# peterropac/Aegolius

Measured on AMD Instinct MI355X. Metric: Mpoints/sec SDF eval, 1024^3 grid, 10-prim smooth-union tree, higher is better.
Workload: dtype f32

## Files before the change

__graft_entry__.py:

```python
import os
import subprocess
import sys

ROOT = os.path.dirname(os.path.abspath(__file__))
CSRC = os.path.join(ROOT, "aegolius_amd", "csrc")
LIB = os.path.join(ROOT, "aegolius_amd", "libsdfk.so")
HELPER = os.path.join(ROOT, "aegolius_amd", "sdfk_rtc_helper")
HELPER_SRC = os.path.join(CSRC, "sdfk_rtc_helper.c")
SOURCES = ["sdfk.hip", "sdfk_codegen.cpp"]
DEPS = SOURCES + ["sdfk_device.h", "sdfk_access.h", "sdfk_codegen.h", "sdfk_ops.def", "sdfk_jit.inc", "sdfk_launch.inc", "sdfk_gridops.inc", "sdfk_fieldops.inc", "sdfk_vector.inc", "sdfk_vecdev.h",
                  "sdfk_hosttree.inc", "sdfk_lcwg.inc", "sdfk_dual.inc", "sdfk_project.inc", "sdfk_dualdev.h", "sdfk_adjoint.inc", "sdfk_points.inc", "sdfk_mesh.inc", "sdfk_slices.inc", "sdfk_topology.inc", "sdfk_rays.inc", "sdfk_raydev.h", "sdfk_raycull.h", "sdfk_interpfield.h", "sdfk_occupancy.inc", "sdfk_occdev.h", "sdfk_moments.inc", "sdfk_momdev.h", "sdfk_redistance.inc", "sdfk_boxdev.h", "sdfk_enclosure.inc", "embed.py",
                  os.path.join("..", "_mctable.py"),
                  os.path.join("..", "..", "include", "sdfk.h")]
HIPCC_FLAGS = ["--offload-arch=gfx950", "-O3", "-ffp-contract=off", "-fno-honor-nans", "-mno-amdgpu-ieee", "-std=c++17",
               "-fPIC", "-shared"]


def _stale():
    if not os.path.exists(LIB):
        return True
    t = os.path.getmtime(LIB)
    return any(os.path.getmtime(os.path.join(CSRC, d)) > t for d in DEPS)


def _write_mesh_table():
    import importlib.util
    spec = importlib.util.spec_from_file_location("_sdfk_mctable", os.path.join(ROOT, "aegolius_amd", "_mctable.py"))
    mod = importlib.util.module_from_spec(spec)
    spec.loader.exec_module(mod)
    mod.write_inc(os.path.join(CSRC, "sdfk_mesh_table.inc"))


def build(force=False):
    if ROOT not in sys.path:
        sys.path.insert(0, ROOT)
    if force or _stale():
        hipcc = os.environ.get("HIPCC") or "/opt/rocm/bin/hipcc"
        if not os.path.exists(hipcc):
            hipcc = "hipcc"
        sys.path.insert(0, CSRC)
        try:
            import embed
            embed.main()
        finally:
# ... 66 lines not shown
```

aegolius_amd/csrc/embed.py:

```python
import os
import sys


def main(out_path=None):
    here = os.path.dirname(os.path.abspath(__file__))
    out_path = out_path or os.path.join(here, "sdfk_embedded.inc")
    parts = []
    for var, name in (("kEmbeddedDevice", "sdfk_device.h"), ("kEmbeddedAccess", "sdfk_access.h"),
                      ("kEmbeddedVecdev", "sdfk_vecdev.h"), ("kEmbeddedRaydev", "sdfk_raydev.h"),
                      ("kEmbeddedRaycull", "sdfk_raycull.h"), ("kEmbeddedOccdev", "sdfk_occdev.h"),
                      ("kEmbeddedMomdev", "sdfk_momdev.h")):
        text = open(os.path.join(here, name)).read()
        assert ')SDFKSRC"' not in text
        parts.append('static const char %s[] = R"SDFKSRC(\n%s\n)SDFKSRC";\n' % (var, text))
    new = "// generated by embed.py - do not edit\n" + "\n".join(parts)
    if not os.path.exists(out_path) or open(out_path).read() != new:
        with open(out_path, "w") as f:
            f.write(new)
    return out_path


if __name__ == "__main__":
    main(*sys.argv[1:])
```

aegolius_amd/csrc/sdfk.hip:

```cpp
#include <hip/hip_runtime.h>
#include <hip/hiprtc.h>

#include <chrono>
#include <algorithm>
#include <atomic>
#include <cmath>
#include <condition_variable>
#include <cstdio>
#include <cstdlib>
#include <cstring>
#include <deque>
#include <functional>
#include <map>
#include <memory>
#include <mutex>
#include <thread>
#include <string>
#include <variant>
#include <vector>
#include <dirent.h>
#include <dlfcn.h>
#include <fcntl.h>
#include <signal.h>
#include <spawn.h>
// ... 676 lines not shown
    const double step = delta / div;
    for (int64_t i = 0; i < n; ++i) {
        volatile double t = (step != 0.0) ? (double)i * step : ((double)i / div) * delta;
        out[i] = (float)(t + lo);
    }
    out[n - 1] = (float)hi;
    return 0;
}

struct AxisTables {
    float* d = nullptr;
    ~AxisTables() {
        if (d) (void)hipFree(d);
    }
};

static int upload_axes(const float* ax0, int64_t n0, const float* ax1, int64_t n1, const float* ax2, int64_t n2,
                       hipStream_t stream, AxisTables* t, SrcGrid* g, int64_t start) {
    if (!ax0 || !ax1 || !ax2 || n0 < 1 || n1 < 1 || n2 < 1) return fail(-1, "grid axes missing or empty");
    if (n1 > 0x7fffffff || n2 > 0x7fffffff) return fail(-1, "grid axis too long");
    HIPCHK(hipMalloc(&t->d, (size_t)(n0 + n1 + n2) * sizeof(float)));
    HIPCHK(hipMemcpyAsync(t->d, ax0, (size_t)n0 * sizeof(float), hipMemcpyHostToDevice, stream));
    HIPCHK(hipMemcpyAsync(t->d + n0, ax1, (size_t)n1 * sizeof(float), hipMemcpyHostToDevice, stream));
    HIPCHK(hipMemcpyAsync(t->d + n0 + n1, ax2, (size_t)n2 * sizeof(float), hipMemcpyHostToDevice, stream));
    g->ax0 = t->d;
    g->ax1 = t->d + n0;
    g->ax2 = t->d + n0 + n1;
    g->n1 = (unsigned)n1;
    g->n2 = (unsigned)n2;
    g->start = start;
    return 0;
}

extern "C" int sdfk_eval_grid_aux(sdfk_program* p, const float* ax0, int64_t n0, const float* ax1, int64_t n1,
                                  const float* ax2, int64_t n2, int64_t start, int64_t count, const float* d_aux, int n_aux,
                                  int64_t aux_stride, float* d_out, void* stream, int mode) {
    if (!p || !d_out) return fail(-1, "sdfk_eval_grid_aux: null pointer");
    if (start < 0 || count < 0 || start + count > n0 * n1 * n2) return fail(-1, "sdfk_eval_grid_aux: range outside the grid");
    if (n_aux < p->n_aux) return fail(-1, "sdfk_eval_grid_aux: the program reads more auxiliary fields than were passed");
    AxisTables t;
    SrcGrid g;
    int rc = upload_axes(ax0, n0, ax1, n1, ax2, n2, (hipStream_t)stream, &t, &g, start);
    if (rc) return rc;
    EvalCall c = grid_call(p, &g, count, d_out, stream, mode, aligned16(d_out));
    c.aux = d_aux;
    c.aux_stride = aux_stride;
    rc = run(c);
    if (rc) return rc;
    HIPCHK(hipStreamSynchronize((hipStream_t)stream));
    return 0;
}
extern "C" int sdfk_eval_grid(sdfk_program* p, const float* ax0, int64_t n0, const float* ax1, int64_t n1,
                              const float* ax2, int64_t n2, int64_t start, int64_t count, float* d_out, void* stream,
                              int mode) {
    if (!d_out) return fail(-1, "sdfk_eval_grid: null output");
    if (start < 0 || count < 0 || start + count > n0 * n1 * n2) return fail(-1, "sdfk_eval_grid: range outside the grid");
    if (!p) return fail(-1, "null program");
    return sdfk_eval_grid_aux(p, ax0, n0, ax1, n1, ax2, n2, start, count, nullptr, p->n_aux, 0, d_out, stream, mode);
}

extern "C" int sdfk_eval_grid_host(sdfk_program* p, const float* ax0, int64_t n0, const float* ax1, int64_t n1,
                                   const float* ax2, int64_t n2, int64_t start, int64_t count, float* out, int device,
                                   int mode) {
    if (!p) return fail(-1, "null program");
    if (count < 0 || (count > 0 && !out)) return fail(-1, "sdfk_eval_grid_host: bad arguments");
    if (start < 0 || start + count > n0 * n1 * n2) return fail(-1, "sdfk_eval_grid_host: range outside the grid");
    if (count == 0) return 0;
    HIPCHK(hipSetDevice(device));
    int64_t chunk = std::min<int64_t>(count, (int64_t)1 << 27);
    const int64_t grow = n2 > 1 ? n2 : n1;
    if (start % grow == 0 && chunk > grow) chunk = chunk / grow * grow;
    float* d_out = nullptr;
    HIPCHK(hipMalloc(&d_out, (size_t)chunk * sizeof(float)));
    AxisTables t;
    SrcGrid g;
// ... 379 lines not shown
```

aegolius_amd/csrc/sdfk_codegen.cpp:

```cpp
#include "sdfk_codegen.h"

#include <algorithm>
#include <cstdio>
#include <cstring>
#include <map>
#include <set>

#include "sdfk_embedded.inc"

std::string sdfk_vector_prelude() { return std::string(kEmbeddedDevice) + "\n" + kEmbeddedVecdev + "\n"; }

static const char kWrappers[] = R"SDFKW(
template <int VEC, typename SRC>
static __device__ __forceinline__ void sdfk_body(const float* __restrict__ PRM, const float* __restrict__ TAB,
                                                 const SRC& src, long long off, long long n,
                                                 float* __restrict__ out, const float* __restrict__ aux,
                                                 long long aux_stride, unsigned* __restrict__ flags, unsigned thr) {
    const long long block_base = (long long)sdfk_bx() * (SDFK_BLOCK * VEC);
    const unsigned lane_off = sdfk_tx() * VEC;
#ifdef SDFK_FLAGS                                              // the flag-writing build of this flavour (its own code object:
    {                                                          // carried as a run-time branch it cost the field kernels registers)
        const bool active = block_base + lane_off < n;
        unsigned nib = 0u;
        if (active) {
// ... 1455 lines not shown
        bool run = false;
        unsigned rec = 0u;
        if (j < cnt) {
            rec = listed ? cp.cand[off + j] : sdfk_member_record(j);
            const float e = SDFK_CHAIN_SGN * sdfk_leaf_rec<float>(rec, c, PRM, TAB);
            run = !(e - m >= thr0 + 1e-6f * fabsf(e));
        }
        const unsigned long long bits = __ballot(run);
        if (run) cp.cand[at + n_out + (unsigned)__builtin_popcountll(bits & ((1ull << lane) - 1ull))] = rec;
        n_out += (unsigned)__builtin_popcountll(bits);
    }
    if (lane == 0) cp.span[cell] = make_uint2(at, total);
}
#else
#define SDFK_CELLS_KARG
#endif
)SDFKR";
static const char kRowsArray[] = R"SDFKR(
extern "C" __global__ __launch_bounds__(64 * SDFK_RWAVES) SDFK_ROWS_ATTR void sdfk_spec_r(
    const float* __restrict__ PRM, const float* __restrict__ TAB, const float* __restrict__ co, long long stride,
    sdfk_rowgeom g, float* __restrict__ out, unsigned* __restrict__ flags, unsigned thr SDFK_CELLS_KARG) {
    const SrcArray s = {co, stride};
    sdfk_rows_kernel(PRM, TAB, s, g, out, flags, thr SDFK_CELLS_PASS);
}
#ifdef SDFK_CELLS
extern "C" __global__ __launch_bounds__(256) void sdfk_spec_cells(
    const float* __restrict__ PRM, const float* __restrict__ TAB, const float* __restrict__ co, long long stride,
    sdfk_rowgeom g, sdfk_cellpass cp) {
    const SrcArray s = {co, stride};
    sdfk_cells_kernel(PRM, TAB, s, g, cp);
}
#endif
)SDFKR";
static const char kRowsGrid[] = R"SDFKR(
// the same on a regular grid expanded from three per-axis tables (no coordinate array: 4 B/point); the slab
// starts at a row boundary and out[0] is its first point
extern "C" __global__ __launch_bounds__(64 * SDFK_RWAVES) void sdfk_spec_rg(
    const float* __restrict__ PRM, const float* __restrict__ TAB, SrcGrid s, sdfk_rowgeom g, float* __restrict__ out,
    unsigned* __restrict__ flags, unsigned thr SDFK_CELLS_KARG) {
    sdfk_rows_kernel(PRM, TAB, s, g, out, flags, thr SDFK_CELLS_PASS);
}
#ifdef SDFK_CELLS
extern "C" __global__ __launch_bounds__(256) void sdfk_spec_cellsg(
    const float* __restrict__ PRM, const float* __restrict__ TAB, SrcGrid s, sdfk_rowgeom g, sdfk_cellpass cp) {
    sdfk_cells_kernel(PRM, TAB, s, g, cp);
}
#endif
)SDFKR";
static const char kRowsMask[] = R"SDFKR(
// test aid: the skip masks (two 64-bit words per brick: sites 0-31, 32-63; bit 2k = first operand of site k
// skipped, bit 2k+1 = second) followed by the "uniform rows" flag in a third word
extern "C" __global__ __launch_bounds__(64 * SDFK_RWAVES) void sdfk_spec_rmask(
    const float* __restrict__ PRM, const float* __restrict__ TAB, const float* __restrict__ co, long long stride,
    sdfk_rowgeom g, unsigned long long* __restrict__ masks) {
    __shared__ __attribute__((aligned(16))) sdfk_rowmeta meta;
    const SrcArray s = {co, stride};
    unsigned rb, c;
    sdfk_rows_prepare(PRM, TAB, s, g, &meta, sdfk_bx(), rb, c);
    const unsigned q = sdfk_bx() * SDFK_RNBRICK + sdfk_tx();
    if (sdfk_tx() < SDFK_RNBRICK && q < g.nbricks) {
        masks[3ull * q] = meta.mask[0][sdfk_tx()];
        masks[3ull * q + 1] = meta.mask[1][sdfk_tx()];
        masks[3ull * q + 2] = meta.uniform[sdfk_tx()];
    }
}
)SDFKR";

namespace {

struct Gen {
    const sdfk_opinfo* ops;
    int n_ops;
    const uint32_t* code;
// ... 886 lines not shown
        g.s += kSpecField;
        g.s += flavour == SDFK_FL_SPANS ? kSpans : flavour == SDFK_FL_SECONDARY ? kSecondary : kRays;
        if (chain) {
            g.s += "\n#ifndef SDFK_RAYS_CULL_MIN_LEAVES\n#define SDFK_RAYS_CULL_MIN_LEAVES 64    // (measured: DESIGN 4.14 has the table)\n#endif\n"
                   "#if SDFK_NLEAF >= SDFK_RAYS_CULL_MIN_LEAVES\n";
            g.s += kWaveHelpers;
            g.s += kEmbeddedRaycull;
            g.s += flavour == SDFK_FL_SPANS ? kSpansCullKernels : flavour == SDFK_FL_SECONDARY ? kSecondaryCullKernels : kRaysCullKernels;
            g.s += "#endif\n";
        }
        return g.s;
    }
    if (chain_analyse(g, result_reg, sites_all)) {
        const bool flat2 = flavour == SDFK_FL_ROWS2D_ARRAY || flavour == SDFK_FL_ROWS2D_GRID;
        g.emit_chain_common();
        if (plain) {
            g.s += kWrappers;
            if (all || flavour == SDFK_FL_PLAIN_ARRAY) g.s += kWrappersArray;
            if (all || flavour == SDFK_FL_PLAIN_GRID) g.s += kWrappersGrid;
        }
        if (all || flat2 || flavour == SDFK_FL_ROWS_ARRAY || flavour == SDFK_FL_ROWS_GRID || flavour == SDFK_FL_ROWS_MASK) {
            g.s += kWaveHelpers;
            if (flat2) g.s += "\n#define SDFK_FLAT 1\n";
            g.s += "\n#define SDFK_NP 4\n#define SDFK_EACH _Pragma(\"unroll\") for (int q = 0; q < SDFK_NP; ++q)\n"
                   "#define SDFK_NMASK 2\n"
                   "#define SDFK_SIMT 1\n#define SDFK_NSUB 1\n"
                   "#ifndef SDFK_CELLS_MIN_LEAVES\n#define SDFK_CELLS_MIN_LEAVES 64\n#endif\n"
                   "#if !defined(SDFK_NO_CELLS) && SDFK_NLEAF > SDFK_CELLS_MIN_LEAVES\n#define SDFK_CELLS 1\n#endif\n"
                   "#ifndef SDFK_LEAF_UNROLL\n#define SDFK_LEAF_UNROLL _Pragma(\"unroll 4\")\n#endif\n";
            g.s += kSimtGeometry;
            g.emit_probe_leaves(g.leaves.size() >= 128, true);
            g.s += kRowsKernel;
            if (all || flavour == SDFK_FL_ROWS_ARRAY || flavour == SDFK_FL_ROWS2D_ARRAY) g.s += kRowsArray;
            if (all || flavour == SDFK_FL_ROWS_GRID || flavour == SDFK_FL_ROWS2D_GRID) g.s += kRowsGrid;
        }
        return g.s;
    }
    if (plain) {
        g.s += "\ntemplate <typename T> static __device__ __forceinline__ T sdfk_point(V3T<T> C_0, "
               "const float* __restrict__ PRM, const float* __restrict__ TAB, const float* __restrict__ AUX, "
               "long long AUXS) {\n";
        g.declare("V3T<T>", "T", false);
        for (size_t i = 0; i < n_instr; ++i) g.instr(i, "    ");
        snprintf(buf, sizeof buf, "    return V_%d;\n}\n", result_reg);
        g.s += buf;
        g.s += kWrappers;
        if (all || flavour == SDFK_FL_PLAIN_ARRAY) g.s += kWrappersArray;
        if (all || flavour == SDFK_FL_PLAIN_GRID) g.s += kWrappersGrid;
    }
    if (tile || rowk) g.s += kWaveHelpers;
    if (tile) {
        std::vector<size_t> order(sites.size());
        for (size_t i = 0; i < order.size(); ++i) order[i] = i;
        std::stable_sort(order.begin(), order.end(), [&](size_t x, size_t y) {
            return sites[x].comb - sites[x].a0 > sites[y].comb - sites[y].a0;
        });
        order.resize(std::min<size_t>(order.size(), 31));
        std::sort(order.begin(), order.end());
        std::vector<sdfk_cullsite> flat;
        for (size_t i : order) flat.push_back(sites[i]);
        g.sites = &flat;
        g.find_roots();
        snprintf(buf, sizeof buf, "\n#define SDFK_NROOT %d\n", g.n_root > 0 ? g.n_root : 1);
        g.s += buf;
        g.emit_probe();
        g.emit_culled(result_reg);
        g.s += kTileKernel;
// ... 8 lines not shown
        g.n_root = 0;
        g.find_roots();
        if (flat) g.s += "\n#define SDFK_FLAT 1\n";
        g.s += "\n#define SDFK_NP 4\n#define SDFK_EACH _Pragma(\"unroll\") for (int q = 0; q < SDFK_NP; ++q)\n";
        {
            char nm[64];
            snprintf(nm, sizeof nm, "#define SDFK_NMASK %zu\n", std::max<size_t>(2, (sites.size() + 31) / 32));
            g.s += nm;
        }
        g.s += "#ifndef SDFK_CHAIN_LOOP_MIN\n#define SDFK_CHAIN_LOOP_MIN 100000   // chains of at least this many sites run as a loop over the levels that survive\n#endif\n"
               "// the even bits of x, packed into the low 32 bits (wave-uniform: scalar unit)\n"
               "static __device__ __forceinline__ unsigned long long sdfk_even_bits(unsigned long long x) {\n"
               "    x &= 0x5555555555555555ull;\n"
               "    x = (x | (x >> 1)) & 0x3333333333333333ull;\n"
               "    x = (x | (x >> 2)) & 0x0f0f0f0f0f0f0f0full;\n"
               "    x = (x | (x >> 4)) & 0x00ff00ff00ff00ffull;\n"
               "    x = (x | (x >> 8)) & 0x0000ffff0000ffffull;\n"
               "    x = (x | (x >> 16)) & 0x00000000ffffffffull;\n"
               "    return x;\n}\n";
        g.simt = g.analyse_leaves();
        if (g.simt) {
            char def[160];
            snprintf(def, sizeof def, "\n#ifndef SDFK_NOSIMT\n#define SDFK_SIMT 1\n#endif\n#define SDFK_NLEAF %zu\n", g.leaves.size());
            g.s += def;
            g.s += kSimtGeometry;
            g.emit_groups();
            g.emit_probe_leaves();
            g.emit_probe_fold();
        }
        g.emit_probe();
        g.emit_rows_culled(result_reg);
        g.s += kRowsKernel;
        if (all || flavour == SDFK_FL_ROWS_ARRAY || flavour == SDFK_FL_ROWS2D_ARRAY) g.s += kRowsArray;
        if (all || flavour == SDFK_FL_ROWS_GRID || flavour == SDFK_FL_ROWS2D_GRID) g.s += kRowsGrid;
        if (all || flavour == SDFK_FL_ROWS_MASK) g.s += kRowsMask;
    }
    return g.s;
}
```

aegolius_amd/csrc/sdfk_jit.inc:

```
static std::string rtc_cache_dir() {
    static const std::string dir = [] {
        std::string d;
        if (const char* e = getenv("SDFK_CACHE_DIR")) {
            d = e;
            if (d.empty() || d == "off" || d == "0") return std::string();
        } else if (const char* x = getenv("XDG_CACHE_HOME"); x && *x) {
            d = std::string(x) + "/sdfk";
        } else if (const char* h = getenv("HOME"); h && *h) {
            (void)mkdir((std::string(h) + "/.cache").c_str(), 0700);
            d = std::string(h) + "/.cache/sdfk";
        } else {
            return std::string();
        }
        (void)mkdir(d.c_str(), 0700);
        return d;
    }();
    return dir;
}
static std::string rtc_cache_path(const std::string& src, const std::string& opts) {
    const std::string dir = rtc_cache_dir();
    if (dir.empty()) return std::string();
    int major = 0, minor = 0;
    (void)hiprtcVersion(&major, &minor);
    unsigned long long h = 1469598103934665603ull;
// ... 427 lines not shown
    std::lock_guard<std::mutex> lk(e->mu);
    e->build_seconds = dt;
    if (rc == 0) {
        e->co.swap(co);
        e->disk_path = disk_path;
        e->state = 2;
    } else {
        e->error = log;
        e->state = 3;
        e->failed_at = std::chrono::steady_clock::now();
    }
    e->cv.notify_all();
}
template <typename MakeSource>
static std::shared_ptr<CodeObject> code_get(const std::string& key, MakeSource make_source, int rwb, bool wait) {
    std::shared_ptr<CodeObject> e = code_entry(key);
    std::unique_lock<std::mutex> lk(e->mu);
    if (e->state == 3 && std::chrono::steady_clock::now() - e->failed_at > std::chrono::seconds(30)) e->state = 0;
    if (e->state == 0) {
        e->state = 1;
        lk.unlock();
        const std::string src = make_source();
        if (wait || !rtc_helper_available()) {
            code_build(e, src, rwb);
        } else {
            g_builds.post([e, src, rwb] { code_build(e, src, rwb, true); });
        }
        return e;
    }
    if (wait) e->cv.wait(lk, [&] { return e->state != 1; });
    return e;
}
static std::string flavour_key(const sdfk_program* p, int flavour, int rwb, int with_flags = 0) {
    return p->key + "|f" + std::to_string(flavour) + ((with_flags & 1) ? "s" : "") + ((with_flags & 2) ? "x" : "") + "|" + rtc_option_key(rwb);
}
static std::string flavour_source(const sdfk_program* p, int flavour, int with_flags = 0) {
    return std::string((with_flags & 1) ? "#define SDFK_FLAGS 1\n" : "") + ((with_flags & 2) ? "#define SDFK_XY 1\n" : "") +
           sdfk_generate_source(g_ops, SDFK_OP_COUNT, p->code.data(), p->code.size() / 2, p->result_reg, p->sites, flavour,
                                &p->sites_all);
}

extern "C" int sdfk_program_chain_members(const sdfk_program* p) {
    return p && p->chain_mode ? p->chain_members : 0;
}
extern "C" int sdfk_program_compile_check(sdfk_program* p, size_t* code_size) {
    if (!p) return fail(-1, "null program");
    size_t total = 0;
    const int rwb = rows_geo(p);
    for (int f = 0; f < SDFK_FL_COUNT; ++f) {
        if (march_flavour(f)) continue;
        if (f == SDFK_FL_OCCUPANCY) continue;
        if (f == SDFK_FL_MOMENTS) continue;
        if (p->sites.empty() && f != SDFK_FL_PLAIN_ARRAY && f != SDFK_FL_PLAIN_GRID) continue;
        if (p->chain_mode && (f == SDFK_FL_TILE_ARRAY || f == SDFK_FL_TILE_GRID || f == SDFK_FL_TILE_MASK || f == SDFK_FL_ROWS_MASK)) continue;
        std::shared_ptr<CodeObject> e = code_get(flavour_key(p, f, rwb), [&] { return flavour_source(p, f); }, rwb, true);
        if (e->state != 2) return fail(-3, e->error);
        total += e->co.size();
    }
    if (code_size) *code_size = total;
    return 0;
}
extern "C" int sdfk_program_compile_flavour(sdfk_program* p, int flavour, size_t* code_size, double* seconds) {
    if (!p) return fail(-1, "null program");
    int with_flags = 0;
    if (flavour >= 0 && (flavour & SDFK_FLAVOUR_FLAGS)) with_flags |= 1;
    if (flavour >= 0 && (flavour & SDFK_FLAVOUR_XY)) with_flags |= 2;
    if (flavour >= 0) flavour &= ~(SDFK_FLAVOUR_FLAGS | SDFK_FLAVOUR_XY);
    if (flavour < 0 || flavour >= SDFK_FL_COUNT) return fail(-1, "sdfk_program_compile_flavour: unknown flavour");
    if (p->sites.empty() && flavour != SDFK_FL_PLAIN_ARRAY && flavour != SDFK_FL_PLAIN_GRID && !march_flavour(flavour) &&
        flavour != SDFK_FL_OCCUPANCY && flavour != SDFK_FL_MOMENTS)
// ... 156 lines not shown
```

aegolius_amd/csrc/sdfk_launch.inc:

```
static int tile_waves() {
    static int v = [] { const char* e = getenv("SDFK_TWAVES"); int t = e ? atoi(e) : 4; return (t >= 1 && t <= 16) ? t : 4; }();
    const int o = g_twaves_override.load();
    return o ? o : v;
}
static int tile_wbricks() {
    static int v = [] {
        const char* e = getenv("SDFK_WBRICKS");
        int t = e ? atoi(e) : 4;
        if (t < 1 || t > 32) t = 4;
        return t;
    }();
    return v;
}
static int tile_points() { return tile_waves() * tile_wbricks() * 128; }
static int rows_waves(const sdfk_program*) {
    if (const int o = g_rwaves_override.load()) return o;
    return 4;
}
static int rows_wbricks(const sdfk_program* p);
static long long big_program_limit() {
    static const long long v = [] {
        const char* e = getenv("SDFK_BIG_PROGRAM");
        const long long t = e ? atoll(e) : 300;
        return t > 0 ? t : 300;
    }();
    return v;
}
static int rows_geo(const sdfk_program* p) {
    const bool big = p && !p->chain_mode && (long long)(p->code.size() / 2) > big_program_limit();
    return rows_wbricks(p) | (rows_waves(p) << 4) | (big ? 1 << 16 : 0);
}
static int rows_wbricks(const sdfk_program* p) {
// ... 325 lines not shown
    }
    pl.needs_specialised = flags || c.xy;
    pl.variant = (flags ? 1 : 0) | (c.xy ? 2 : 0);
    if (mode == SDFK_MODE_AUTO && n_instr > env.spec_limit && p->interp_ok && !p->chain_mode && !flags)
        mode = SDFK_MODE_INTERPRET;

    const SrcGrid* grid = c.grid;
    pl.flavour = c.arr ? SDFK_FL_PLAIN_ARRAY : SDFK_FL_PLAIN_GRID;
    const long long grow = grid ? (grid->n2 > 1 ? (long long)grid->n2 : (long long)grid->n1) : 0;
    if (!p->sites.empty() && mode != SDFK_MODE_NOCULL && mode != SDFK_MODE_INTERPRET) {
        if (c.arr && rows_geometry(c.n, c.row_len, &pl.rg, (c.flat || flags) ? 0 : c.plane_rows, c.plane_phase, p->chain_mode))
            pl.flavour = (c.flat || c.xy) ? SDFK_FL_ROWS2D_ARRAY : SDFK_FL_ROWS_ARRAY;
        else if (c.arr && c.vec_ok && !p->chain_mode && !flags && !c.xy) pl.flavour = SDFK_FL_TILE_ARRAY;
        else if (grid && grid->start % grow == 0 &&
                 rows_geometry(c.n, grow, &pl.rg, (grid->n2 > 1 && !flags) ? (long long)grid->n1 : 0,
                               grid->n2 > 1 ? (grid->start / grow) % (long long)grid->n1 : 0, p->chain_mode))
            pl.flavour = grid->n2 > 1 ? SDFK_FL_ROWS_GRID : SDFK_FL_ROWS2D_GRID;
        else if (grid && c.vec_ok && !p->chain_mode && !flags) pl.flavour = SDFK_FL_TILE_GRID;
        if (!p->chain_mode && n_instr > env.rows_limit && pl.rows()) {
            const bool is_arr = c.arr != nullptr;
            if (c.vec_ok && !flags && !c.xy) pl.flavour = is_arr ? SDFK_FL_TILE_ARRAY : SDFK_FL_TILE_GRID;
            else if (!flags) pl.flavour = is_arr ? SDFK_FL_PLAIN_ARRAY : SDFK_FL_PLAIN_GRID;
        }
    }
    if (grid && pl.rows()) {
        pl.rg.row0 = grid->start / grow;
        pl.rg.yrows = grid->n2 > 1 ? 0 : 1;
    }
    pl.mode = mode;
    *out = pl;
    return 0;
}

static int launch_specialised(const EvalCall& c, const EvalPlan& pl, const LaunchCtx& x, const SpecModule& sk) {
    sdfk_program* p = c.p;
    const float *prm = x.prm, *tab = x.tab, *aux = c.aux, *co = c.arr ? c.arr->co : nullptr;
    long long n = c.n, aux_stride = c.aux_stride, stride = c.arr ? c.arr->stride : 0;
    float* d_out = c.d_out;
    unsigned* d_flags = c.d_flags;
    unsigned thr_key = c.thr_key;
    SrcGrid g = c.grid ? *c.grid : SrcGrid{};
    void* args[13] = {&prm, &tab, &co, &stride};
    if (c.grid) args[2] = &g;
    const int n_src = c.grid ? 1 : 2;
    auto go = [&](hipFunction_t fn, unsigned blocks, unsigned threads, std::initializer_list<void*> own) {
        std::copy(own.begin(), own.end(), args + 2 + n_src);
        return hipModuleLaunchKernel(fn, blocks, 1, 1, threads, 1, 1, 0, x.stream, args, nullptr);
    };
    if (pl.rows()) {
        RowGeom rg = pl.rg;
        const unsigned per_tile = (unsigned)(rows_waves(p) * rows_wbricks(p));
        const unsigned tiles = ((rg.nbricks + per_tile - 1) / per_tile + 127u) & ~127u;
        CellsArg cells{};
        if (p->chain_mode && sk.fn[1] != nullptr) {
            const int rc = prepare_cells(p, x.d, sk.fn[1], rg, args + 2, n_src, prm, tab, x.stream, &cells);
            if (rc) return rc;
        }
        HIPCHK(go(sk.fn[0], tiles, 64u * (unsigned)rows_waves(p), {&rg, &d_out, &d_flags, &thr_key, &cells}));
    } else if (pl.tile()) {
        HIPCHK(go(sk.fn[0], (unsigned)((n + tile_points() - 1) / tile_points()), tile_threads(), {&n, &d_out}));
    } else {
        long long n4 = c.vec_ok ? (n / 4) * 4 : 0, tail = n - n4, zero = 0;
        if (n4) HIPCHK(go(sk.fn[0], blocks_for(n4, 4), SDFK_BLOCK, {&zero, &n4, &d_out, &aux, &aux_stride, &d_flags, &thr_key}));
        if (tail) HIPCHK(go(sk.fn[1], blocks_for(tail, 1), SDFK_BLOCK, {&n4, &tail, &d_out, &aux, &aux_stride, &d_flags, &thr_key}));
    }
    return 0;
}

static int launch_interpreter(const EvalCall& c, const LaunchCtx& x) {
    const sdfk_program* p = c.p;
    const long long n4 = c.vec_ok ? (c.n / 4) * 4 : 0, tail = c.n - n4, zero = 0;
    auto launch = [&](auto src, int vec, long long off, long long cnt) {
        using SRC = decltype(src);
        const dim3 grid(blocks_for(cnt, vec)), block(SDFK_BLOCK);
#define SDFK_INTERP_GO4(NC, NV) hipLaunchKernelGGL((sdfk_interp_kernel<4, NC, NV, SRC>), grid, block, 0, x.stream, x.d->d_code, \
                                                   x.n_instr, x.prm, x.tab, src, off, cnt, c.d_out, x.result_reg, c.aux, c.aux_stride)
#define SDFK_INTERP_GO1(NC, NV) hipLaunchKernelGGL((sdfk_interp_kernel<1, NC, NV, SRC>), grid, block, 0, x.stream, x.d->d_code, \
                                                   x.n_instr, x.prm, x.tab, src, off, cnt, c.d_out, x.result_reg, c.aux, c.aux_stride)
        if (vec == 4) SDFK_REGFILE(p, SDFK_NC, SDFK_NV, SDFK_INTERP_GO4);
        else SDFK_REGFILE(p, SDFK_NC, SDFK_NV, SDFK_INTERP_GO1);
#undef SDFK_INTERP_GO4
#undef SDFK_INTERP_GO1
    };
    if (c.arr) {
        if (n4) launch(*c.arr, 4, zero, n4);
        if (tail) launch(*c.arr, 1, n4, tail);
    } else {
        if (n4) launch(*c.grid, 4, zero, n4);
        if (tail) launch(*c.grid, 1, n4, tail);
    }
    HIPCHK(hipGetLastError());
    return 0;
}

static int run(const EvalCall& c) {
    sdfk_program* p = c.p;
    if (!p) return fail(-1, "null program");
    if (c.n < 0) return fail(-1, "negative point count");
    if (p->n_aux > 0 && (!c.aux || c.aux_stride < c.n))
        return fail(-1, "this program reads auxiliary fields (staged evaluation): use sdfk_eval_device_aux / sdfk_eval_grid_aux");
    if (c.n == 0) return 0;
    EvalPlan own;
    int rc = c.plan ? 0 : plan_eval(c, plan_env(), &own);
    if (rc) return rc;
    const EvalPlan& pl = c.plan ? *c.plan : own;
    LaunchCtx x;
    rc = launch_ctx(p, c.stream, &x);
    if (rc) return rc;
    std::shared_ptr<SpecModule> sk;
    rc = pick_kernel(p, x.device, pl.flavour, pl.variant, pl.mode, pl.mode != SDFK_MODE_SPECIALIZED && !pl.needs_specialised,
                     "kernel", true, &sk);
    if (rc) return rc;
    return sk ? launch_specialised(c, pl, x, *sk) : launch_interpreter(c, x);
}
```

Before: 367,100.

## Add table-based grid rows kernel and cache uploaded grid axes per device

Adds a new rows-grid kernel path that reads per-axis coordinate tables directly. It computes per-sub-brick probe spheres with exact radii from those tables and culls subtrees with shared-memory skip masks before evaluating and storing whole rows. Grid axes are now kept in a small per-device LRU cache instead of being uploaded and synchronised on every call. The old grid path stays available as a fallback variant when the table geometry does not fit. The cost is more code, extra kernel arguments, host-side memcmp of the axes on each call, and extra codegen complexity.

Result: no change. 366,900 (-0.1%).

```diff
diff --git a/__graft_entry__.py b/__graft_entry__.py
--- a/__graft_entry__.py
+++ b/__graft_entry__.py
@@ -9,7 +9,7 @@
 HELPER_SRC = os.path.join(CSRC, "sdfk_rtc_helper.c")
 SOURCES = ["sdfk.hip", "sdfk_codegen.cpp"]
 DEPS = SOURCES + ["sdfk_device.h", "sdfk_access.h", "sdfk_codegen.h", "sdfk_ops.def", "sdfk_jit.inc", "sdfk_launch.inc", "sdfk_gridops.inc", "sdfk_fieldops.inc", "sdfk_vector.inc", "sdfk_vecdev.h",
-                  "sdfk_hosttree.inc", "sdfk_lcwg.inc", "sdfk_dual.inc", "sdfk_project.inc", "sdfk_dualdev.h", "sdfk_adjoint.inc", "sdfk_points.inc", "sdfk_mesh.inc", "sdfk_slices.inc", "sdfk_topology.inc", "sdfk_rays.inc", "sdfk_raydev.h", "sdfk_raycull.h", "sdfk_interpfield.h", "sdfk_occupancy.inc", "sdfk_occdev.h", "sdfk_moments.inc", "sdfk_momdev.h", "sdfk_redistance.inc", "sdfk_boxdev.h", "sdfk_enclosure.inc", "embed.py",
+                  "sdfk_hosttree.inc", "sdfk_lcwg.inc", "sdfk_dual.inc", "sdfk_project.inc", "sdfk_dualdev.h", "sdfk_adjoint.inc", "sdfk_points.inc", "sdfk_mesh.inc", "sdfk_slices.inc", "sdfk_topology.inc", "sdfk_rays.inc", "sdfk_raydev.h", "sdfk_raycull.h", "sdfk_interpfield.h", "sdfk_occupancy.inc", "sdfk_occdev.h", "sdfk_moments.inc", "sdfk_momdev.h", "sdfk_gridtab.h", "sdfk_redistance.inc", "sdfk_boxdev.h", "sdfk_enclosure.inc", "embed.py",
                   os.path.join("..", "_mctable.py"),
                   os.path.join("..", "..", "include", "sdfk.h")]
 HIPCC_FLAGS = ["--offload-arch=gfx950", "-O3", "-ffp-contract=off", "-fno-honor-nans", "-mno-amdgpu-ieee", "-std=c++17",
diff --git a/aegolius_amd/csrc/embed.py b/aegolius_amd/csrc/embed.py
--- a/aegolius_amd/csrc/embed.py
+++ b/aegolius_amd/csrc/embed.py
@@ -9,7 +9,7 @@
     for var, name in (("kEmbeddedDevice", "sdfk_device.h"), ("kEmbeddedAccess", "sdfk_access.h"),
                       ("kEmbeddedVecdev", "sdfk_vecdev.h"), ("kEmbeddedRaydev", "sdfk_raydev.h"),
                       ("kEmbeddedRaycull", "sdfk_raycull.h"), ("kEmbeddedOccdev", "sdfk_occdev.h"),
-                      ("kEmbeddedMomdev", "sdfk_momdev.h")):
+                      ("kEmbeddedMomdev", "sdfk_momdev.h"), ("kEmbeddedGridtab", "sdfk_gridtab.h")):
         text = open(os.path.join(here, name)).read()
         assert ')SDFKSRC"' not in text
         parts.append('static const char %s[] = R"SDFKSRC(\n%s\n)SDFKSRC";\n' % (var, text))
diff --git a/aegolius_amd/csrc/sdfk.hip b/aegolius_amd/csrc/sdfk.hip
--- a/aegolius_amd/csrc/sdfk.hip
+++ b/aegolius_amd/csrc/sdfk.hip
@@ -732,15 +732,91 @@
     return 0;
 }
 
+struct AxisEntry {
+    int64_t n0 = 0, n1 = 0, n2 = 0;
+    std::vector<float> host;
+    AxisTables dev;
+    unsigned long long used = 0;
+};
+static std::mutex g_axis_mu;
+static std::map<int, std::vector<std::shared_ptr<AxisEntry>>> g_axis_cache;
+static unsigned long long g_axis_clock = 0;
+static const size_t kAxisCacheEntries = 4;
+extern "C" void sdfk_axis_cache_clear(void) {
+    std::map<int, std::vector<std::shared_ptr<AxisEntry>>> gone;
+    {
+        std::lock_guard<std::mutex> lk(g_axis_mu);
+        gone.swap(g_axis_cache);
+    }
+    int cur = 0;
+    const bool have = hipGetDevice(&cur) == hipSuccess;
+    for (auto& kv : gone) {
+        if (hipSetDevice(kv.first) != hipSuccess) continue;
+        kv.second.clear();
+    }
+    if (have) (void)hipSetDevice(cur);
+}
+static int cached_axes(const float* ax0, int64_t n0, const float* ax1, int64_t n1, const float* ax2, int64_t n2,
+                       hipStream_t stream, std::shared_ptr<AxisEntry>* hold, SrcGrid* g, int64_t start) {
+    if (!ax0 || !ax1 || !ax2 || n0 < 1 || n1 < 1 || n2 < 1) return fail(-1, "grid axes missing or empty");
+    if (n1 > 0x7fffffff || n2 > 0x7fffffff) return fail(-1, "grid axis too long");
+    int device = 0;
+    HIPCHK(hipGetDevice(&device));
+    std::shared_ptr<AxisEntry> e;
+    {
+        std::lock_guard<std::mutex> lk(g_axis_mu);
+        for (const std::shared_ptr<AxisEntry>& c : g_axis_cache[device])
+            if (c->n0 == n0 && c->n1 == n1 && c->n2 == n2 && memcmp(c->host.data(), ax0, (size_t)n0 * sizeof(float)) == 0 &&
+                memcmp(c->host.data() + n0, ax1, (size_t)n1 * sizeof(float)) == 0 &&
+                memcmp(c->host.data() + n0 + n1, ax2, (size_t)n2 * sizeof(float)) == 0) {
+                e = c;
+                e->used = ++g_axis_clock;
+                break;
+            }
+    }
+    if (!e) {
+        e = std::make_shared<AxisEntry>();
+        e->n0 = n0; e->n1 = n1; e->n2 = n2;
+        e->host.resize((size_t)(n0 + n1 + n2));
+        memcpy(e->host.data(), ax0, (size_t)n0 * sizeof(float));
+        memcpy(e->host.data() + n0, ax1, (size_t)n1 * sizeof(float));
+        memcpy(e->host.data() + n0 + n1, ax2, (size_t)n2 * sizeof(float));
+        HIPCHK(hipMalloc(&e->dev.d, e->host.size() * sizeof(float)));
+        HIPCHK(hipMemcpyAsync(e->dev.d, e->host.data(), e->host.size() * sizeof(float), hipMemcpyHostToDevice, stream));
+        HIPCHK(hipStreamSynchronize(stream));
+        std::shared_ptr<AxisEntry> out;
+        std::lock_guard<std::mutex> lk(g_axis_mu);
+        std::vector<std::shared_ptr<AxisEntry>>& v = g_axis_cache[device];
+        e->used = ++g_axis_clock;
+        if (v.size() >= kAxisCacheEntries) {
+            size_t lru = 0;
+            for (size_t i = 1; i < v.size(); ++i)
+                if (v[i]->used < v[lru]->used) lru = i;
+            out = v[lru];
+            v[lru] = e;
+        } else {
+            v.push_back(e);
+        }
+    }
+    g->ax0 = e->dev.d;
+    g->ax1 = e->dev.d + n0;
+    g->ax2 = e->dev.d + n0 + n1;
+    g->n1 = (unsigned)n1;
+    g->n2 = (unsigned)n2;
+    g->start = start;
+    *hold = e;
+    return 0;
+}
+
 extern "C" int sdfk_eval_grid_aux(sdfk_program* p, const float* ax0, int64_t n0, const float* ax1, int64_t n1,
                                   const float* ax2, int64_t n2, int64_t start, int64_t count, const float* d_aux, int n_aux,
                                   int64_t aux_stride, float* d_out, void* stream, int mode) {
     if (!p || !d_out) return fail(-1, "sdfk_eval_grid_aux: null pointer");
     if (start < 0 || count < 0 || start + count > n0 * n1 * n2) return fail(-1, "sdfk_eval_grid_aux: range outside the grid");
     if (n_aux < p->n_aux) return fail(-1, "sdfk_eval_grid_aux: the program reads more auxiliary fields than were passed");
-    AxisTables t;
+    std::shared_ptr<AxisEntry> t;
     SrcGrid g;
-    int rc = upload_axes(ax0, n0, ax1, n1, ax2, n2, (hipStream_t)stream, &t, &g, start);
+    int rc = cached_axes(ax0, n0, ax1, n1, ax2, n2, (hipStream_t)stream, &t, &g, start);
     if (rc) return rc;
     EvalCall c = grid_call(p, &g, count, d_out, stream, mode, aligned16(d_out));
     c.aux = d_aux;
diff --git a/aegolius_amd/csrc/sdfk_codegen.cpp b/aegolius_amd/csrc/sdfk_codegen.cpp
--- a/aegolius_amd/csrc/sdfk_codegen.cpp
+++ b/aegolius_amd/csrc/sdfk_codegen.cpp
@@ -1511,13 +1511,235 @@
 }
 #endif
 )SDFKR";
+static const char kRowsGridTab[] = R"SDFKR(
+#if defined(SDFK_SIMT) && !defined(SDFK_CHAIN) && !defined(SDFK_CELLS) && !defined(SDFK_FLAGS) && !defined(SDFK_FLAT) && \
+    !defined(SDFK_GRID_OLD) && SDFK_NP == 4
+#define SDFK_GRID_TAB 1
+struct sdfk_tabmeta {
+    float4 cen[SDFK_NCEN];                      // probe centres (x, y, z, radius): SDFK_NSUB per brick
+    float leafval[SDFK_NLEAF * SDFK_NCEN];      // [leaf][centre]
+    unsigned long long mask[SDFK_NMASK][SDFK_RNBRICK];
+};
+// lanes that share the rows of one probe centre (consecutive lanes of one wave)
+#define SDFK_TAB_PL ((64 * SDFK_RWAVES) / SDFK_NCEN >= 4 ? 4 : ((64 * SDFK_RWAVES) / SDFK_NCEN >= 2 ? 2 : 1))
+// rows of a sub-brick unless a plane change cuts the block elsewhere (sdfk_tab_sub)
+#define SDFK_TAB_RPS (SDFK_NSUB >= 4 ? 16 / (SDFK_NSUB / 4) : 16)
+// elements [z, z + 8) of a row from the third table: whole quads inside an interior window (rows need only 4-byte
+// alignment), else element by element, the nearest point of the row for those outside it
+static __device__ __forceinline__ void sdfk_tab_z8(const SrcGrid& s, const sdfk_tabgeom& t, int z, bool interior, float (&v)[8]) {
+    if (interior) {
+        const sdfk_f4u a = *reinterpret_cast<const sdfk_f4u*>(s.ax2 + z), b = *reinterpret_cast<const sdfk_f4u*>(s.ax2 + z + 4);
+        v[0] = a.x; v[1] = a.y; v[2] = a.z; v[3] = a.w; v[4] = b.x; v[5] = b.y; v[6] = b.z; v[7] = b.w;
+    } else {
+#pragma unroll
+        for (int i = 0; i < 8; ++i) v[i] = s.ax2[sdfk_tab_zclamp(t, z + i)];
+    }
+}
+// Probe centre cn of the tile, lane `part` of its SDFK_TAB_PL: the sub-brick's sphere around the midpoint of its first
+// and last point; the radius is the exact maximum over its points, whatever the tables hold (no order, no spacing is
+// assumed): a sub-brick is rows x window elements, a row has one x and one y, so per row
+// |p - c|^2 = (x - cx)^2 + (y - cy)^2 + max_i (z_i - cz)^2. (The elements of a window are different points of the third
+// axis in every row unless L is a multiple of 32: every row reads its own.) Same inflation as sdfk_sub_centre.
+static __device__ __forceinline__ float4 sdfk_tab_centre(const SrcGrid& s, const sdfk_tabgeom& t, unsigned tile, unsigned cn,
+                                                         unsigned part) {
+    const unsigned b = cn / SDFK_NSUB, sb = cn % SDFK_NSUB;
+    unsigned r0, rend, c;
+    float cx = 0.0f, cy = 0.0f, cz = 0.0f, r2 = 0.0f;
+    // (a padded tile or a dead brick forms no table index: harmless values for the probe lane that still meets it)
+    const bool live = sdfk_tab_live(t, tile * SDFK_RNBRICK + b, &r0, &rend, &c);
+    if (live) {
+        unsigned s0, s1, i0, zps, ixa, iya, ixe, iye;
+        long long f;
+        sdfk_tab_sub(t, SDFK_NSUB, sb, r0, rend - r0, &s0, &s1, &i0, &zps);
+        const bool interior = sdfk_tab_interior(t, c);
+        sdfk_tab_xy(t, r0 + s0, &ixa, &iya);
+        sdfk_tab_xy(t, r0 + s1 - 1u, &ixe, &iye);
+        const int za = sdfk_tab_win(t, r0 + s0, c, i0, &f), ze = sdfk_tab_win(t, r0 + s1 - 1u, c, i0 + zps - 1u, &f);
+        cx = 0.5f * (s.ax0[ixa] + s.ax0[ixe]);
+        cy = 0.5f * (s.ax1[iya] + s.ax1[iye]);
+        cz = 0.5f * (s.ax2[sdfk_tab_zclamp(t, za)] + s.ax2[sdfk_tab_zclamp(t, ze)]);
+#ifdef SDFK_ABLATE_BOUNDS                                        // (timing only: half the diagonal, too small for sheared windows)
+        {
+            const float ex = s.ax0[ixe] - cx, ey = s.ax1[iye] - cy, ez = s.ax2[sdfk_tab_zclamp(t, ze)] - cz;
+            r2 = sd_fma(ez, ez, sd_fma(ex, ex, ey * ey));
+        }
+#else
+        // the usual part — 8 window elements of at most SDFK_TAB_RPS rows — with a fixed trip count: every load of the
+        // lane (centre and rows) is in flight at once, one memory round trip before the barrier instead of one per row
+        constexpr unsigned IT = (SDFK_TAB_RPS + SDFK_TAB_PL - 1) / SDFK_TAB_PL;
+        if (SDFK_NSUB >= 4 && s1 - s0 <= SDFK_TAB_RPS) {
+            float xr[IT], yr[IT], zr[IT][8];
+#pragma unroll
+            for (unsigned it = 0; it < IT; ++it) {
+                unsigned r = s0 + part + it * SDFK_TAB_PL, ix, iy;
+                if (r >= s1) r = s1 - 1u;                         // (a row twice: the maximum does not care)
+                sdfk_tab_xy(t, r0 + r, &ix, &iy);
+                xr[it] = s.ax0[ix];
+                yr[it] = s.ax1[iy];
+                const int z = sdfk_tab_win(t, r0 + r, c, i0, &f);
+                sdfk_tab_z8(s, t, z, interior, zr[it]);
+            }
+#pragma unroll
+            for (unsigned it = 0; it < IT; ++it) {
+                const float dx = xr[it] - cx, dy = yr[it] - cy;
+                float zm = 0.0f;
+#pragma unroll
+                for (int i = 0; i < 8; ++i) zm = sd_rawmax(zm, sd_abs(zr[it][i] - cz));
+                r2 = sd_rawmax(r2, sd_fma(zm, zm, sd_fma(dx, dx, dy * dy)));
+            }
+        } else {
+#pragma unroll 1
+            for (unsigned r = s0 + part; r < s1; r += SDFK_TAB_PL) {
+                unsigned ix, iy;
+                sdfk_tab_xy(t, r0 + r, &ix, &iy);
+                const float dx = s.ax0[ix] - cx, dy = s.ax1[iy] - cy;
+                const int z = sdfk_tab_win(t, r0 + r, c, i0, &f);
+                float zm = 0.0f;
+#pragma unroll 1
+                for (unsigned i = 0; i < zps; i += 8u) {
+                    float z8[8];
+                    sdfk_tab_z8(s, t, z + (int)i, interior, z8);
+#pragma unroll
+                    for (int e = 0; e < 8; ++e) zm = sd_rawmax(zm, sd_abs(z8[e] - cz));
+                }
+                r2 = sd_rawmax(r2, sd_fma(zm, zm, sd_fma(dx, dx, dy * dy)));
+            }
+        }
+#endif
+    }
+    if (SDFK_TAB_PL >= 2) r2 = sd_rawmax(r2, __shfl_xor(r2, 1));
+    if (SDFK_TAB_PL >= 4) r2 = sd_rawmax(r2, __shfl_xor(r2, 2));
+    return make_float4(cx, cy, cz, live ? 1.00001f * sqrtf(r2) + 1e-30f : 1.0f);
+}
+// Phase C of one brick (wave-uniform q): a lane owns 2 * SDFK_NP consecutive window elements of ONE row. First its
+// coordinates — x and y of its row, its elements of the third table —, then the culled body and the stores.
+struct sdfk_tabpts {
+    bool live, interior, live_row;
+    int z;                                      // index in the row of the lane's first point (edge windows: may lie outside)
+    long long f;                                // its output index
+    float x, y;
+    f2 zz[SDFK_NP];
+};
+static __device__ __forceinline__ void sdfk_tab_fetch(const SrcGrid& s, const sdfk_tabgeom& t, unsigned q, unsigned lr, unsigned zq,
+                                                      sdfk_tabpts& p) {
+    unsigned r0, rend, k;
+    p.live = sdfk_tab_live(t, q, &r0, &rend, &k);
+    if (!p.live) return;                                          // padded tile, dead brick: no index is formed
+    p.interior = sdfk_tab_interior(t, k);
+#ifdef SDFK_ABLATE_EDGE
+    if (!p.interior) { p.live = false; return; }
+#endif
+    p.live_row = r0 + lr < rend;
+    const unsigned row = sdfk_tab_row(r0, rend, lr);
+    p.z = sdfk_tab_win(t, row, k, zq, &p.f);
+    unsigned ix, iy;
+    sdfk_tab_xy(t, row, &ix, &iy);
+    p.x = s.ax0[ix];
+    p.y = s.ax1[iy];
+    float z8[8];                                                  // (outside the row: the nearest point of it, never stored)
+    sdfk_tab_z8(s, t, p.z, p.interior, z8);
+    SDFK_EACH p.zz[q] = {z8[2 * q], z8[2 * q + 1]};
+}
+static __device__ __forceinline__ void sdfk_tab_brick_eval(const float* __restrict__ PRM, const float* __restrict__ TAB,
+                                                           const sdfk_tabgeom& t,
+                                                           const unsigned long long (&mask)[SDFK_NMASK][SDFK_RNBRICK], unsigned b,
+                                                           const sdfk_tabpts& p, float* __restrict__ out) {
+    unsigned mw[2 * SDFK_NMASK];                                 // the brick's skip bits as scalar words
+#pragma unroll
+    for (int w = 0; w < SDFK_NMASK; ++w) {
+        const unsigned long long m = mask[w][b];
+        mw[2 * w] = __builtin_amdgcn_readfirstlane((unsigned)m);
+        mw[2 * w + 1] = __builtin_amdgcn_readfirstlane((unsigned)(m >> 32));
+    }
+    V3P P[SDFK_NP];
+    f2 res[SDFK_NP];
+    SDFK_EACH { P[q].x = sp<f2>(p.x); P[q].y = sp<f2>(p.y); P[q].z = p.zz[q]; }
+#ifdef SDFK_ABLATE_EVAL
+    SDFK_EACH res[q] = P[q].z + __builtin_bit_cast(float, mw[0] ^ mw[1] ^ mw[2] ^ mw[3]);
+#else
+    sdfk_rows_culled<true>(p.x, p.y, P, mw, PRM, TAB, res);
+#endif
+    if (p.live_row) {
+        float* po = out + p.f;
+        if (p.interior) {
+#pragma unroll
+            for (int q = 0; q < SDFK_NP; q += 2) {
+                sdfk_f4u v = {res[q].x, res[q].y, res[q + 1].x, res[q + 1].y};
+                __builtin_nontemporal_store(v, reinterpret_cast<sdfk_f4u*>(po + 2 * q));
+            }
+        } else {
+            SDFK_EACH {
+                if (sdfk_tab_inrow(t, p.z + 2 * q)) po[2 * q] = res[q].x;
+                if (sdfk_tab_inrow(t, p.z + 2 * q + 1)) po[2 * q + 1] = res[q].y;
+            }
+        }
+    }
+}
+static __device__ __forceinline__ void sdfk_rows_tab_kernel(const float* __restrict__ PRM, const float* __restrict__ TAB,
+                                                            const SrcGrid& s, const sdfk_tabgeom& t, float* __restrict__ out) {
+    __shared__ __attribute__((aligned(16))) sdfk_tabmeta meta;
+    const unsigned tx = sdfk_tx();
+    const unsigned lane = tx & 63u, wave = __builtin_amdgcn_readfirstlane(tx >> 6);
+    const unsigned lr = lane / SDFK_RLPR, zq = (lane % SDFK_RLPR) * (2 * SDFK_NP);
+#pragma unroll 1
+  for (unsigned tt = 0; tt < SDFK_RTILES; ++tt) {
+    // (runs of SDFK_XGROUP consecutive tiles per XCD, as in sdfk_rows_kernel)
+    const unsigned tile = sdfk_tab_tile(sdfk_bx(), SDFK_XGROUP) * SDFK_RTILES + tt;
+    if (tile * SDFK_RNBRICK >= t.nbricks) break;                // the launch is rounded up: nothing is read or written
+    if (tt) __syncthreads();
+    // the probe: centres -> every leaf at every centre (all lanes) -> one fold lane per centre ANDs its skip decisions
+    // into the brick's mask (a subtree is skipped only if every sub-brick allows it)
+    if (tx < SDFK_RNBRICK) {
+#pragma unroll
+#ifdef SDFK_ABLATE_PROBE
+        for (int w = 0; w < SDFK_NMASK; ++w) meta.mask[w][tx] = 0ull;      // (no probe: nothing is skipped)
+#else
+        for (int w = 0; w < SDFK_NMASK; ++w) meta.mask[w][tx] = ~0ull;
+#endif
+    }
+    if (tx < SDFK_NCEN * SDFK_TAB_PL) {
+        const float4 cc = sdfk_tab_centre(s, t, tile, tx / SDFK_TAB_PL, tx % SDFK_TAB_PL);
+        if (tx % SDFK_TAB_PL == 0u) meta.cen[tx / SDFK_TAB_PL] = cc;
+    }
+    __syncthreads();
+#ifndef SDFK_ABLATE_PROBE
+    sdfk_probe_leaves(meta.cen, meta.leafval, PRM, TAB);
+    __syncthreads();
+    if (tx < SDFK_NCEN && tile * SDFK_RNBRICK + tx / SDFK_NSUB < t.nbricks) {
+        const float4 cc = meta.cen[tx];
+        V3T<float> ctr = {cc.x, cc.y, cc.z};
+        unsigned long long mk[SDFK_NMASK];
+        sdfk_probe_fold(meta.leafval, tx, ctr, cc.w, PRM, mk);
+#pragma unroll
+        for (int w = 0; w < SDFK_NMASK; ++w)
+            __hip_atomic_fetch_and(&meta.mask[w][tx / SDFK_NSUB], mk[w], __ATOMIC_RELAXED, __HIP_MEMORY_SCOPE_WORKGROUP);
+    }
+    __syncthreads();
+#endif
+    const unsigned q0 = tile * SDFK_RNBRICK + wave * SDFK_RWBRICKS;
+#pragma unroll 1
+    for (unsigned j = 0; j < SDFK_RWBRICKS; ++j) {
+        sdfk_tabpts pt;
+        sdfk_tab_fetch(s, t, q0 + j, lr, zq, pt);
+        if (!pt.live) continue;                                   // (wave-uniform)
+        sdfk_tab_brick_eval(PRM, TAB, t, meta.mask, wave * SDFK_RWBRICKS + j, pt, out);
+    }
+  }
+}
+#endif
+)SDFKR";
 static const char kRowsGrid[] = R"SDFKR(
 // the same on a regular grid expanded from three per-axis tables (no coordinate array: 4 B/point); the slab
-// starts at a row boundary and out[0] is its first point
+// starts at a row boundary and out[0] is its first point. tg: the geometry of the axis-table skeleton (sdfk_gridtab.h),
+// which the builds that have it run instead of sdfk_rows_kernel
 extern "C" __global__ __launch_bounds__(64 * SDFK_RWAVES) void sdfk_spec_rg(
     const float* __restrict__ PRM, const float* __restrict__ TAB, SrcGrid s, sdfk_rowgeom g, float* __restrict__ out,
-    unsigned* __restrict__ flags, unsigned thr SDFK_CELLS_KARG) {
+    unsigned* __restrict__ flags, unsigned thr, sdfk_tabgeom tg SDFK_CELLS_KARG) {
+#ifdef SDFK_GRID_TAB
+    sdfk_rows_tab_kernel(PRM, TAB, s, tg, out);
+#else
     sdfk_rows_kernel(PRM, TAB, s, g, out, flags, thr SDFK_CELLS_PASS);
+#endif
 }
 #ifdef SDFK_CELLS
 extern "C" __global__ __launch_bounds__(256) void sdfk_spec_cellsg(
@@ -2470,7 +2692,11 @@
             g.emit_probe_leaves(g.leaves.size() >= 128, true);
             g.s += kRowsKernel;
             if (all || flavour == SDFK_FL_ROWS_ARRAY || flavour == SDFK_FL_ROWS2D_ARRAY) g.s += kRowsArray;
-            if (all || flavour == SDFK_FL_ROWS_GRID || flavour == SDFK_FL_ROWS2D_GRID) g.s += kRowsGrid;
+            if (all || flavour == SDFK_FL_ROWS_GRID || flavour == SDFK_FL_ROWS2D_GRID) {
+                g.s += kEmbeddedGridtab;
+                g.s += kRowsGridTab;
+                g.s += kRowsGrid;
+            }
         }
         return g.s;
     }
@@ -2545,7 +2771,11 @@
         g.emit_rows_culled(result_reg);
         g.s += kRowsKernel;
         if (all || flavour == SDFK_FL_ROWS_ARRAY || flavour == SDFK_FL_ROWS2D_ARRAY) g.s += kRowsArray;
-        if (all || flavour == SDFK_FL_ROWS_GRID || flavour == SDFK_FL_ROWS2D_GRID) g.s += kRowsGrid;
+        if (all || flavour == SDFK_FL_ROWS_GRID || flavour == SDFK_FL_ROWS2D_GRID) {
+            g.s += kEmbeddedGridtab;
+            g.s += kRowsGridTab;
+            g.s += kRowsGrid;
+        }
         if (all || flavour == SDFK_FL_ROWS_MASK) g.s += kRowsMask;
     }
     return g.s;
diff --git a/aegolius_amd/csrc/sdfk_gridtab.h b/aegolius_amd/csrc/sdfk_gridtab.h
--- /dev/null
+++ b/aegolius_amd/csrc/sdfk_gridtab.h
@@ -0,0 +1,122 @@
+#ifndef SDFK_GRIDTAB_H
+#define SDFK_GRIDTAB_H
+
+#if defined(__HIP__) || defined(__HIPCC__) || defined(__HIPCC_RTC__)
+#define SDFK_TAB_FN static __host__ __device__ __forceinline__
+#else
+#define SDFK_TAB_FN static inline
+#endif
+
+#define SDFK_TAB_ROWS 16u
+#define SDFK_TAB_WIN 32u
+
+struct sdfk_tabgeom {
+    unsigned L, nchunk, nbricks, R;
+    unsigned prow, seg0, nb0, bpp;
+    unsigned inv_nchunk, inv_bpp, inv_n1, n1;
+    unsigned ix0, iy0;
+    unsigned one_plane, pad;
+};
+
+SDFK_TAB_FN unsigned sdfk_tab_inv(unsigned long long d) {
+    const unsigned long long v = (1ull << 32) / (d ? d : 1ull);
+    return v > 0xffffffffull ? 0xffffffffu : (unsigned)v;
+}
+SDFK_TAB_FN unsigned sdfk_tab_div(unsigned a, unsigned d, unsigned inv) {
+    unsigned q = (unsigned)(((unsigned long long)a * inv) >> 32);
+    unsigned r = a - q * d;
+    if (r >= d) { ++q; r -= d; }
+    if (r >= d) ++q;
+    return q;
+}
+SDFK_TAB_FN bool sdfk_tab_setup(sdfk_tabgeom* t, unsigned L, unsigned nchunk, unsigned nbricks, long long R, long long row0,
+                                unsigned prow, unsigned seg0, unsigned nb0, unsigned bpp, unsigned n1) {
+    if (n1 == 0u || R <= 0 || row0 < 0 || R + (long long)n1 + 64 > 0x7fffffffLL || row0 / (long long)n1 > 0x7fffffffLL) return false;
+    t->L = L; t->nchunk = nchunk; t->nbricks = nbricks; t->R = (unsigned)R;
+    t->prow = prow; t->seg0 = seg0; t->nb0 = nb0; t->bpp = bpp;
+    t->inv_nchunk = sdfk_tab_inv(nchunk); t->inv_bpp = sdfk_tab_inv(bpp); t->inv_n1 = sdfk_tab_inv(n1); t->n1 = n1;
+    t->ix0 = (unsigned)(row0 / (long long)n1); t->iy0 = (unsigned)(row0 % (long long)n1);
+    t->one_plane = (nb0 == 0u && (long long)prow >= R) ? 1u : 0u;
+    t->pad = 0u;
+    return true;
+}
+
+SDFK_TAB_FN void sdfk_tab_brick(const sdfk_tabgeom& t, unsigned q, unsigned* rb, unsigned* c) {
+    *rb = sdfk_tab_div(q, t.nchunk, t.inv_nchunk);
+    *c = q - *rb * t.nchunk;
+}
+SDFK_TAB_FN void sdfk_tab_block(const sdfk_tabgeom& t, unsigned rb, unsigned* r0, unsigned* rend) {
+    if (t.one_plane) {
+        *r0 = rb * SDFK_TAB_ROWS;
+        *rend = t.R;
+    } else if (rb < t.nb0) {
+        *r0 = rb * SDFK_TAB_ROWS;
+        *rend = t.seg0;
+    } else {
+        const unsigned k = rb - t.nb0;
+        const unsigned pl = sdfk_tab_div(k, t.bpp, t.inv_bpp);
+        const unsigned base = t.seg0 + pl * t.prow;
+        *r0 = base + (k - pl * t.bpp) * SDFK_TAB_ROWS;
+        *rend = base + t.prow < t.R ? base + t.prow : t.R;
+    }
+    if (*r0 > *rend) *r0 = *rend;
+    if (*rend - *r0 > SDFK_TAB_ROWS) *rend = *r0 + SDFK_TAB_ROWS;
+}
+SDFK_TAB_FN bool sdfk_tab_live(const sdfk_tabgeom& t, unsigned q, unsigned* r0, unsigned* rend, unsigned* c) {
+    *r0 = *rend = *c = 0u;
+    if (q >= t.nbricks) return false;
+    unsigned rb;
+    sdfk_tab_brick(t, q, &rb, c);
+    sdfk_tab_block(t, rb, r0, rend);
+    return *r0 < *rend;
+}
+SDFK_TAB_FN unsigned sdfk_tab_row(unsigned r0, unsigned rend, unsigned dr) {
+    return r0 + dr < rend ? r0 + dr : rend - 1u;
+}
+SDFK_TAB_FN void sdfk_tab_xy(const sdfk_tabgeom& t, unsigned row, unsigned* ix, unsigned* iy) {
+    const unsigned a = t.iy0 + row;
+    const unsigned pl = sdfk_tab_div(a, t.n1, t.inv_n1);
+    *ix = t.ix0 + pl;
+    *iy = a - pl * t.n1;
+}
+SDFK_TAB_FN int sdfk_tab_win(const sdfk_tabgeom& t, unsigned row, unsigned k, unsigned e0, long long* flat) {
+    const long long rl = (long long)row * (long long)t.L;
+    const long long f = (((rl >> 5) + (long long)k) << 5) + (long long)e0;
+    *flat = f;
+    return (int)(f - rl);
+}
+SDFK_TAB_FN bool sdfk_tab_interior(const sdfk_tabgeom& t, unsigned k) {
+    return (t.L & 31u) == 0u || (k >= 1u && 32u * k + 32u <= t.L);
+}
+SDFK_TAB_FN bool sdfk_tab_inrow(const sdfk_tabgeom& t, int z) { return z >= 0 && z < (int)t.L; }
+SDFK_TAB_FN unsigned sdfk_tab_zclamp(const sdfk_tabgeom& t, int z) {
+    return (unsigned)(z < 0 ? 0 : (z >= (int)t.L ? (int)t.L - 1 : z));
+}
+SDFK_TAB_FN unsigned sdfk_tab_tile(unsigned bx, unsigned xgroup) {
+    const unsigned t = bx / 8u;
+    return ((t / xgroup) * 8u + bx % 8u) * xgroup + t % xgroup;
+}
+SDFK_TAB_FN void sdfk_tab_sub(const sdfk_tabgeom& t, unsigned nsub, unsigned sb, unsigned r0, unsigned nrows, unsigned* s0,
+                              unsigned* s1, unsigned* i0, unsigned* zps) {
+    const unsigned nzp = nsub >= 4u ? 4u : 1u, nrp = nsub / nzp, rps = SDFK_TAB_ROWS / nrp;
+    *zps = SDFK_TAB_WIN / nzp;
+    *i0 = (sb % nzp) * *zps;
+    unsigned a = (sb / nzp) * rps, b = a + rps;
+    if (nrp == 2u) {
+        unsigned ixa, ixb, iy;
+        sdfk_tab_xy(t, r0, &ixa, &iy);
+        sdfk_tab_xy(t, r0 + nrows - 1u, &ixb, &iy);
+        if (ixa != ixb) {
+            const unsigned cut = t.n1 - (t.iy0 + r0 - (ixa - t.ix0) * t.n1);
+            a = sb / nzp ? cut : 0u;
+            b = sb / nzp ? SDFK_TAB_ROWS : cut;
+        }
+    }
+    if (a > nrows - 1u) a = nrows - 1u;
+    if (b > nrows) b = nrows;
+    if (b <= a) b = a + 1u;
+    *s0 = a;
+    *s1 = b;
+}
+
+#endif
diff --git a/aegolius_amd/csrc/sdfk_jit.inc b/aegolius_amd/csrc/sdfk_jit.inc
--- a/aegolius_amd/csrc/sdfk_jit.inc
+++ b/aegolius_amd/csrc/sdfk_jit.inc
@@ -483,10 +483,12 @@
     return e;
 }
 static std::string flavour_key(const sdfk_program* p, int flavour, int rwb, int with_flags = 0) {
-    return p->key + "|f" + std::to_string(flavour) + ((with_flags & 1) ? "s" : "") + ((with_flags & 2) ? "x" : "") + "|" + rtc_option_key(rwb);
+    return p->key + "|f" + std::to_string(flavour) + ((with_flags & 1) ? "s" : "") + ((with_flags & 2) ? "x" : "") + ((with_flags & 4) ? "o" : "") + "|" +
+           rtc_option_key(rwb);
 }
 static std::string flavour_source(const sdfk_program* p, int flavour, int with_flags = 0) {
     return std::string((with_flags & 1) ? "#define SDFK_FLAGS 1\n" : "") + ((with_flags & 2) ? "#define SDFK_XY 1\n" : "") +
+           ((with_flags & 4) ? "#define SDFK_GRID_OLD 1\n" : "") +
            sdfk_generate_source(g_ops, SDFK_OP_COUNT, p->code.data(), p->code.size() / 2, p->result_reg, p->sites, flavour,
                                 &p->sites_all);
 }
diff --git a/aegolius_amd/csrc/sdfk_launch.inc b/aegolius_amd/csrc/sdfk_launch.inc
--- a/aegolius_amd/csrc/sdfk_launch.inc
+++ b/aegolius_amd/csrc/sdfk_launch.inc
@@ -1,3 +1,4 @@
+#include "sdfk_gridtab.h"
 static int tile_waves() {
     static int v = [] { const char* e = getenv("SDFK_TWAVES"); int t = e ? atoi(e) : 4; return (t >= 1 && t <= 16) ? t : 4; }();
     const int o = g_twaves_override.load();
@@ -389,6 +390,12 @@
     return 0;
 }
 
+static bool grid_tab_geometry(const EvalCall& c, const EvalPlan& pl, sdfk_tabgeom* tg) {
+    memset(tg, 0, sizeof *tg);
+    if (!c.grid || pl.flavour != SDFK_FL_ROWS_GRID || (pl.variant & 1) || pl.rg.yrows || pl.rg.L != c.grid->n2) return false;
+    return sdfk_tab_setup(tg, pl.rg.L, pl.rg.nchunk, pl.rg.nbricks, pl.rg.R, pl.rg.row0, pl.rg.prow, pl.rg.seg0, pl.rg.nb0, pl.rg.bpp,
+                          c.grid->n1);
+}
 static int launch_specialised(const EvalCall& c, const EvalPlan& pl, const LaunchCtx& x, const SpecModule& sk) {
     sdfk_program* p = c.p;
     const float *prm = x.prm, *tab = x.tab, *aux = c.aux, *co = c.arr ? c.arr->co : nullptr;
@@ -413,7 +420,13 @@
             const int rc = prepare_cells(p, x.d, sk.fn[1], rg, args + 2, n_src, prm, tab, x.stream, &cells);
             if (rc) return rc;
         }
-        HIPCHK(go(sk.fn[0], tiles, 64u * (unsigned)rows_waves(p), {&rg, &d_out, &d_flags, &thr_key, &cells}));
+        if (c.grid) {
+            sdfk_tabgeom tg;
+            (void)grid_tab_geometry(c, pl, &tg);
+            HIPCHK(go(sk.fn[0], tiles, 64u * (unsigned)rows_waves(p), {&rg, &d_out, &d_flags, &thr_key, &tg, &cells}));
+        } else {
+            HIPCHK(go(sk.fn[0], tiles, 64u * (unsigned)rows_waves(p), {&rg, &d_out, &d_flags, &thr_key, &cells}));
+        }
     } else if (pl.tile()) {
         HIPCHK(go(sk.fn[0], (unsigned)((n + tile_points() - 1) / tile_points()), tile_threads(), {&n, &d_out}));
     } else {
@@ -465,7 +478,12 @@
     rc = launch_ctx(p, c.stream, &x);
     if (rc) return rc;
     std::shared_ptr<SpecModule> sk;
-    rc = pick_kernel(p, x.device, pl.flavour, pl.variant, pl.mode, pl.mode != SDFK_MODE_SPECIALIZED && !pl.needs_specialised,
+    int variant = pl.variant;
+    {
+        sdfk_tabgeom tg;
+        if (pl.flavour == SDFK_FL_ROWS_GRID && !(variant & 1) && !grid_tab_geometry(c, pl, &tg)) variant |= 4;
+    }
+    rc = pick_kernel(p, x.device, pl.flavour, variant, pl.mode, pl.mode != SDFK_MODE_SPECIALIZED && !pl.needs_specialised,
                      "kernel", true, &sk);
     if (rc) return rc;
     return sk ? launch_specialised(c, pl, x, *sk) : launch_interpreter(c, x);
```
